# goalheart/ionic-mpnn

Hardware: AMD Instinct MI355X
Metric: molecule-graph pairs/sec (fwd), batch 4096 per MI355X (higher is better)
Workload: dtype f32 (bf16x9 emulation)

## Files before the change

### ionic_mpnn_amd/csrc/encoder_layout.h

```cpp
#pragma once

#include "common.h"

namespace impnn {
namespace enc {

typedef float f32x4 __attribute__((ext_vector_type(4)));
typedef _Float16 half8 __attribute__((ext_vector_type(8)));

constexpr float kSW = 256.0f;
constexpr float kSX = 16.0f;
constexpr float kAcc = kSW * kSX;

constexpr int kD = 32;
constexpr int kKMax = 8;
constexpr int kRCap = 256;
constexpr int kECap = 1024;
constexpr int kHS = 36;
constexpr int kMsgRS = 36;
constexpr int kUpdRS = 68;
constexpr int kThreads = 1024;
constexpr int kWaves = kThreads / 64;
constexpr int kTbCapFloats = 2048;

__host__ __device__ constexpr int img_msg_floats(int K) { return K * kD * kMsgRS; }
__host__ __device__ constexpr int img_upd_floats() { return 3 * kD * kUpdRS; }
__host__ __device__ constexpr int img_vec_floats() { return 5 * kD; }
__host__ __device__ constexpr int img_floats(int K) {
  return img_msg_floats(K) + img_upd_floats() + img_vec_floats();
}
__host__ __device__ constexpr int img16_msg_halfs(int K) { return K * 2 * 2 * 512; }
__host__ __device__ constexpr int img16_upd_halfs() { return 3 * 2 * 2 * 2 * 512; }
__host__ __device__ constexpr int img16_vec_float_off(int K) { return (img16_msg_halfs(K) + img16_upd_halfs()) / 2; }
__host__ __device__ constexpr int feat_of(int q, int j) { return 16 * (j >> 2) + 4 * q + (j & 3); }
constexpr int kPf = 4;
constexpr int kImgSlot = kPf * kThreads * 4;
static_assert(kThreads == 4 * kRCap, "prologue maps 4 threads to a row");
static_assert(img_floats(kKMax) <= kImgSlot, "weight image does not fit its slot");
static_assert(img16_vec_float_off(kKMax) + img_vec_floats() <= kImgSlot, "split weight image does not fit");

constexpr int kRecRowptr = 0;
constexpr int kRecTilemax = 528;
constexpr int kRecMoloff = 544;
constexpr int kRecMolrows = 1072;
constexpr int kRecPoolrow = 1584;
constexpr int kRecRowatom = 2096;
constexpr int kEntMaxAtom = 454;
constexpr int kRecEnt = 3136;
constexpr int kRecBytes = 8192;
static_assert(kRecEnt + 4 * kECap <= kRecBytes && kRecEnt % 16 == 0, "record layout");

constexpr int kTECap = 512;
constexpr int kTECapBig = 640;
__host__ __device__ constexpr int tecap_of(int E) { return E > kTECap ? kTECapBig : kTECap; }
constexpr int kTVbMax = 256;
constexpr int kTHS = 36;
constexpr int kTAS = 32;
constexpr int kTRecRowdeg = 0;
constexpr int kTRecTilemax = 528;
constexpr int kTRecMoloff = 544;
constexpr int kTRecMolrows = 1072;
constexpr int kTRecPoolrow = 1584;
constexpr int kTRecRowatom = 2096;
constexpr int kTRecCounts = 3120;
constexpr int kTRecJdptr = 3136;
constexpr int kTRecNrun = 3664;
constexpr int kTRecGrp = 3712;
constexpr int kTRunTarget = 32;
__host__ __device__ constexpr int tgrp_cap(int Vb, int ecap) { return ecap / 4 + (Vb < kTVbMax ? Vb : kTVbMax); }
__host__ __device__ constexpr int trec_runs_off(int Vb, int ecap) { return kTRecGrp + 16 * tgrp_cap(Vb, ecap); }
__host__ __device__ constexpr int trec_used_bytes(int Vb, int ecap) {
  return (trec_runs_off(Vb, ecap) + 2 * (Vb + 2 + kTRunTarget) + 15) & ~15;
}
constexpr int kTRecBytes = 12288;
constexpr int kTRecPart1 = 8192;
__host__ __device__ constexpr int trec_lds_bytes(int Vb, int ecap) { return trec_used_bytes(Vb, ecap); }
static_assert(kTRecGrp % 16 == 0 && trec_used_bytes(kTVbMax, kTECapBig) <= kTRecBytes, "typed record layout");
__host__ __device__ constexpr int tmsg_floats(int ecap) { return (ecap + 2) * kD; }
__host__ __device__ constexpr int tmsg_off(int s, int u) { return s * kD + ((u ^ ((s >> 1) & 7)) << 2); }
__host__ __device__ constexpr int tmsg_key(int s) { return s * kD + (((s >> 1) & 7) << 2); }
static_assert(tmsg_key(kTECapBig + 1) < 65536, "message keys travel as 16 bits");
constexpr int kTUpdBlocks = 24;
constexpr int kTVecFloatOff = kTUpdBlocks * 256;
constexpr int kTUpdFloats = kTVecFloatOff + 5 * kD;
constexpr int kTUpdSlot = 2 * kThreads * 4;
constexpr int kTUpdLds = 6400;
static_assert(kTUpdFloats <= kTUpdLds && kTUpdLds <= kTUpdSlot, "typed update image");
constexpr int kXUpdHalfs = 3 * 2 * 2 * 3 * 512;
constexpr int kXVecFloatOff = kXUpdHalfs / 2;
constexpr int kXUpdFloats = kXVecFloatOff + 5 * kD;
constexpr int kXUpdSlot = 3 * kThreads * 4;
constexpr int kXUpdLds = 9472;
static_assert(kXUpdFloats <= kXUpdLds && kXUpdLds <= kXUpdSlot, "x3 update image");
constexpr int kTMatFloats = kD * kD;
inline size_t typed_prepared_floats(int S, int Vb, bool x3 = false) {
  const size_t s = S > 0 ? S : 1;
  return s * (x3 ? kXUpdSlot : kTUpdSlot) + s * (size_t)Vb * kTMatFloats + (size_t)Vb * kTMatFloats;
}

constexpr int kShareCap = kECap;
inline int plan_vmin(int n_ions, int B, int vrmax, int nwg) {
  const int64_t span = 2 * (int64_t)n_ions * B * vrmax / (nwg > 0 ? nwg : 1) + vrmax;
  const int64_t v = (span + kShareCap - 2) / (kShareCap - 1);
  return (int)(v < 1 ? 1 : (v > kRCap ? kRCap : v));
}
constexpr int kMaxHops = 128;

constexpr int kPB = 16;

struct Ws {
  size_t img_off, rows_off, vr_off, partial_off, share_off, nsub_off, desc_off, rec_off, total;
  int nwg;
  int max_sub;
  int nblk;
  int rec_bytes;
};

inline size_t align_up(size_t x, size_t a) { return (x + a - 1) / a * a; }

__host__ __device__ constexpr int tvr_of_edges(int edges, int ecap) { return (edges * kRCap + ecap - 1) / ecap; }

inline int vr_max_of(int N, int E, bool typed = false) {
  int v = typed ? (E > 4 * kTECapBig ? kRCap + 1 : tvr_of_edges(E, tecap_of(E))) : (E + 3) / 4;
  int m = N > v ? N : v;
  m = m < 1 ? 1 : m;
  return typed && m > kRCap ? kRCap : m;
}

struct PlanHeader {
  int32_t magic, kind, n_ions, B, N, E, nwg, max_sub;
  int32_t overflow;
};
constexpr int32_t kPlanMagic = 0x696d706e;
constexpr int32_t kPlanBadBit = 1 << 30;

inline Ws ws_layout(int n_ions, int B, int N, int E, int S, int Vb, int nwg, bool typed, bool x3 = false) {
  Ws w{};
  const int vrmax = vr_max_of(N, E, typed);
  w.rec_bytes = typed ? kTRecBytes : kRecBytes;
  const int win = kRCap - vrmax + 1;
  w.nwg = nwg;
  w.nblk = (B + kPB - 1) / kPB;
  const int64_t share_rows = (2 * (int64_t)n_ions * B * vrmax) / nwg + vrmax;
  const int64_t by_win = win >= 1 ? share_rows / win + 2 : (int64_t)1 << 40;
  const int64_t by_pairs = 2 * share_rows / (kRCap + 1) + 2;
  w.max_sub = (int)(by_win < by_pairs ? by_win : by_pairs);
  size_t off = 256;
  w.img_off = off;
  off = align_up(off + (typed ? (size_t)n_ions * typed_prepared_floats(S, Vb, x3)
                              : (size_t)n_ions * (S > 0 ? S : 1) * kImgSlot) * sizeof(float), 256);
  w.rows_off = off;
  off = align_up(off + (size_t)n_ions * B * sizeof(int32_t), 256);
  w.vr_off = off;
  off = align_up(off + (size_t)n_ions * B * sizeof(int32_t), 256);
  w.partial_off = off;
  off = align_up(off + (size_t)n_ions * w.nblk * sizeof(int32_t), 256);
  w.share_off = off;
  off = align_up(off + (size_t)nwg * 4 * sizeof(int32_t), 256);
  w.nsub_off = off;
  off = align_up(off + (size_t)nwg * sizeof(int32_t), 256);
  w.desc_off = off;
  off = align_up(off + (size_t)nwg * w.max_sub * 4 * sizeof(int32_t), 256);
  w.rec_off = off;
  off = align_up(off + (size_t)nwg * w.max_sub * w.rec_bytes, 256);
  w.total = off;
  return w;
}

struct PlanParams {
  const int32_t* atom_ids[2];
  const int32_t* bond_ids[2];
  const int32_t* conn[2];
  int32_t* rows;
  int32_t* vr;
  int32_t* partial;
  int32_t* nsub;
  int32_t* desc;
  unsigned char* rec;
  int n_ions, B, N, E, Va, Vb, nwg, max_sub, nblk;
  int grid_sub;
  int typed;
  int ecap;
  int vmin;
  PlanHeader* header;
  unsigned long long* stamps;
};

struct ImageParams {
  const float* weights;
  float* img;
  int K, mode;
  int64_t step_floats;
};

struct EncParams {
  const int32_t* atom_ids[2];
  float* pooled[2];
  const float* atom_table;
  const float* bond_table;
  const float* img[2];
  const int32_t* nsub;
  const int32_t* desc;
  const unsigned char* rec;
  const PlanHeader* header;
  int n_ions, B, N, K, S, Va, Vb, max_sub;
  int atab_lds;
  float ln_eps;
  unsigned long long* stamps;
};

struct TImageParams {
  const float* weights;
  const float* bond_table;
  float* prepared;
  int K, S, Vb, x3;
  int64_t step_floats;
};

struct TEncParams {
  float* pooled[2];
  const float* atom_table;
  const float* upd[2];
  const float* tmat[2];
  const int32_t* nsub;
  const int32_t* desc;
// ... 36 lines not shown
```

### ionic_mpnn_amd/csrc/encoder_plan.hip

```cpp
#include "encoder_layout.h"

namespace impnn {
namespace enc {

namespace {

__global__ __launch_bounds__(64 * kPB) void plan_stats_kernel(PlanParams p) {
  __shared__ int vsum[kPB], vbad[kPB];
  __builtin_amdgcn_s_setprio(3);
  const int lane = threadIdx.x & 63, wv = threadIdx.x >> 6;
  const int g = blockIdx.x / p.nblk, blk = blockIdx.x - g * p.nblk;
  const int b = blk * kPB + wv;
  const bool have = b < p.B;
  const int64_t item = (int64_t)g * p.B + (have ? b : 0);
  int my_vr = 0, my_bad = 0;
  if (have) {
  const int32_t* ids = p.atom_ids[g] + (int64_t)b * p.N;
  const int32_t* cn = p.conn[g] + (int64_t)b * p.E * 2;
  const int32_t* bd = p.bond_ids[g] + (int64_t)b * p.E;
  int rmax = 0, cnt = 0;
  const int id_first = lane < p.N ? ids[lane] : 0;
  int emax = 0;
  for (int e0 = 0; e0 < p.E; e0 += 256) {
    int2 st[4];
// ... 728 lines not shown
    const int slot = tid + k * kRCap;
    sid[k] = slot < n_ids ? ids_c[slot] : 0;
  }
  for (int m = tid; m <= M; m += kRCap) {
    const int off = T.shst[mb_local + m] - base;
    moloff[m] = off;
    r_moloff[m] = (uint16_t)off;
    if (m < M) {
      const int rr = rows_g[m0 + m];
      molrows[m] = rr;
      r_molrows[m] = (uint16_t)rr;
    }
  }
  cnt[tid] = 0;
  dbins[tid] = 0;
  dcur[tid] = 0;
  thist[tid] = 0;
  tcur[tid] = 0;
  idl[tid] = -1;
  if (tid == 0) misc[1] = 0;
  {
    const uint4 ones = make_uint4(~0u, ~0u, ~0u, ~0u);
    reinterpret_cast<uint4*>(tick)[2 * tid] = ones;
    reinterpret_cast<uint4*>(tick)[2 * tid + 1] = ones;
  }
  lds_barrier();
  CSTAMP(2);

  auto put_id = [&](int slot, int id) {
    const int m = fast_div(slot, N, rN), n = slot - m * N;
    if (slot < n_ids && n < molrows[m]) idl[moloff[m] + n] = id;
  };
  {
    const int dq = fast_div(kRCap, N, rN), dr = kRCap - dq * N;
    int cm = fast_div(tid, N, rN), cn = tid - cm * N;
    int mr[kIC], mo[kIC], nn[kIC];
#pragma unroll
    for (int k = 0; k < kIC; ++k) {
      const int mm = tid + k * kRCap < n_ids ? cm : 0;
      mr[k] = tid + k * kRCap < n_ids ? molrows[mm] : 0;
      mo[k] = moloff[mm];
      nn[k] = cn;
      cn += dr; cm += dq;
      if (cn >= N) { cn -= N; ++cm; }
    }
#pragma unroll
    for (int k = 0; k < kIC; ++k)
      if (nn[k] < mr[k]) idl[mo[k] + nn[k]] = sid[k];
  }
  for (int slot = tid + kIC * kRCap; slot < n_ids; slot += kRCap) put_id(slot, ids_c[slot]);
  {
    unsigned okm = 0u;
#pragma unroll
    for (int k = 0; k < kSC; ++k) okm |= edge_valid(sst[k].x, sst[k].y, sbid[k], N, p.Vb) ? 1u << k : 0u;
    const int mine = __builtin_popcount(okm);
    const int incl = wave_incl_scan(mine);
    int pos = 0;
    if (lane == 63) pos = atomicAdd(&misc[1], incl);
    pos = __builtin_amdgcn_readlane(pos, 63) + incl - mine;
    const int dq = fast_div(kRCap, E, rE), dr = kRCap - dq * E;
    int cm = fast_div(tid, E, rE), ce = tid - cm * E;
#pragma unroll
    for (int k0 = 0; k0 < kSC; k0 += 3) {
      int row[3], srw[3], tk[3], es[3];
#pragma unroll
      for (int k = 0; k < 3; ++k) {
        const bool ok = (okm >> (k0 + k)) & 1u;
        const int m = cm;
        es[k] = ce;
        ce += dr; cm += dq;
        if (ce >= E) { ce -= E; ++cm; }
        const int mo = moloff[m < M ? m : 0];
        row[k] = mo + (ok ? sst[k0 + k].y : 0);
        srw[k] = mo + (ok ? sst[k0 + k].x : 0);
      }
#pragma unroll
      for (int k = 0; k < 3; ++k) {
        const bool ok = (okm >> (k0 + k)) & 1u;
        tk[k] = atomicAdd(&cnt[ok ? row[k] : kRCap + lane], 1);
        atomicAdd(&thist[ok ? sbid[k0 + k] : kTVbMax + lane], 1);
      }
#pragma unroll
      for (int k = 0; k < 3; ++k) {
        const bool ok = (okm >> (k0 + k)) & 1u;
        if (ok && tk[k] < kTick) tick[row[k] * kTick + tk[k]] = (uint16_t)es[k];
        if (ok) {
          if (pos < kTECapBig)
            elist[pos] = make_uint2((uint32_t)row[k] | ((uint32_t)srw[k] << 8) | ((uint32_t)sbid[k0 + k] << 16), (uint32_t)es[k]);
          ++pos;
        }
      }
    }
  }
  for (int s0 = kSC * kRCap; s0 < n_slots; s0 += kRCap) {
    const int slot = s0 + tid;
    int2 st = make_int2(0, 0);
    int bid = -1;
    if (slot < n_slots) {
      st = *reinterpret_cast<const int2*>(conn_c + 2 * (int64_t)slot);
      bid = bond_c[slot];
    }
    const bool ok = edge_valid(st.x, st.y, bid, N, p.Vb);
    const int m = fast_div(slot, E, rE), e = slot - m * E;
    const int mo = moloff[m < M ? m : 0];
    const int row = mo + (ok ? st.y : 0);
    int tk = kTick;
    if (ok) {
      tk = atomicAdd(&cnt[row], 1);
      atomicAdd(&thist[bid], 1);
    }
    const unsigned long long okb = __ballot(ok);
    int pos0 = 0;
    if (okb != 0ull) {
      if (lane == (int)__builtin_ctzll(okb)) pos0 = atomicAdd(&misc[1], (int)__builtin_popcountll(okb));
      pos0 = __builtin_amdgcn_readlane(pos0, (int)__builtin_ctzll(okb));
    }
    if (tk < kTick) tick[row * kTick + tk] = (uint16_t)e;
    const int pos = pos0 + (int)__builtin_popcountll(okb & ((1ull << lane) - 1));
    if (ok && pos < kTECapBig)
      elist[pos] = make_uint2((uint32_t)row | ((uint32_t)(mo + st.x) << 8) | ((uint32_t)bid << 16), (uint32_t)e);
  }
  lds_barrier();
  CSTAMP(3);

  const int my_deg = cnt[tid];
  const int dcl = my_deg > 255 ? 255 : my_deg;
  if (tid < R) {
    if (my_deg > 255) p.header->overflow = 1;
    atomicAdd(&dbins[255 - dcl], 1);
  }
  lds_barrier();
  CSTAMP(4);

  if (wave == 0) {
    const int4 h = reinterpret_cast<const int4*>(dbins)[lane];
    const int s4 = h.x + h.y + h.z + h.w;
    const int ex = wave_incl_scan(s4) - s4;
    reinterpret_cast<int4*>(dstart)[lane] = make_int4(ex, ex + h.x, ex + h.x + h.y, ex + h.x + h.y + h.z);
    __builtin_amdgcn_s_waitcnt(0xc07f);
    const int4 s = reinterpret_cast<const int4*>(dstart)[63 - lane];
    const int t4 = s.x + s.y + s.z + s.w;
    const int incl = wave_incl_scan(t4);
    const int jx = incl - t4;
    reinterpret_cast<int4*>(jdp)[lane] = make_int4(jx, jx + s.w, jx + s.w + s.z, jx + s.w + s.z + s.y);
    if (lane == 63) { jdp[kRCap] = incl; jdp[kRCap + 1] = incl; }
  } else if (wave == 1) {
    const int4 n = reinterpret_cast<const int4*>(thist)[lane];
    const int4 ng = make_int4((n.x + 3) >> 2, (n.y + 3) >> 2, (n.z + 3) >> 2, (n.w + 3) >> 2);
    const int s4 = ng.x + ng.y + ng.z + ng.w;
    const int incl = wave_incl_scan(s4);
    const int ex = incl - s4;
    reinterpret_cast<int4*>(tgb)[lane] = make_int4(ex, ex + ng.x, ex + ng.x + ng.y, ex + ng.x + ng.y + ng.z);
    const int ngrp_all = __builtin_amdgcn_readlane(incl, 63);
    int gmax = (ngrp_all + kTRunTarget - 1) / kTRunTarget;
    gmax = gmax < 2 ? 2 : gmax;
    const float rgm = 1.0f / (float)gmax;
    const int4 nr = make_int4(fast_div(ng.x + gmax - 1, gmax, rgm), fast_div(ng.y + gmax - 1, gmax, rgm),
                              fast_div(ng.z + gmax - 1, gmax, rgm), fast_div(ng.w + gmax - 1, gmax, rgm));
    const int r4 = nr.x + nr.y + nr.z + nr.w;
    const int rincl = wave_incl_scan(r4);
    int ri = rincl - r4;
    uint16_t* runs = reinterpret_cast<uint16_t*>(rec + trec_runs_off(p.Vb, p.ecap));
    for (int i = 0; i < nr.x; ++i) runs[ri++] = (uint16_t)(ex + i * gmax);
    for (int i = 0; i < nr.y; ++i) runs[ri++] = (uint16_t)(ex + ng.x + i * gmax);
    for (int i = 0; i < nr.z; ++i) runs[ri++] = (uint16_t)(ex + ng.x + ng.y + i * gmax);
    for (int i = 0; i < nr.w; ++i) runs[ri++] = (uint16_t)(ex + ng.x + ng.y + ng.z + i * gmax);
    if (lane == 63) {
      runs[rincl] = (uint16_t)incl;
      *reinterpret_cast<uint16_t*>(rec + kTRecNrun) = (uint16_t)rincl;
      misc[0] = incl;
    }
  }
  lds_barrier();
  CSTAMP(5);

  int pos = tid;
  if (tid < R) pos = dstart[255 - dcl] + atomicAdd(&dcur[255 - dcl], 1);
  place[tid] = pos;
  {
    const int my_id = idl[tid];
    r_rowatom[pos] = my_id;
    r_poolrow[tid] = (uint16_t)(pos | (my_id > 0 ? 0x8000 : 0));
    r_rowdeg[pos] = (uint16_t)my_deg;
    if ((pos & 15) == 0) r_tilemax[pos >> 4] = (unsigned char)dcl;
    r_jd[tid] = (uint16_t)jdp[tid];
    if (tid < 2) r_jd[kRCap + tid] = (uint16_t)jdp[kRCap];
    if (pos == 0) {
      r_cw[0] = (uint16_t)misc[0];
      r_cw[1] = (uint16_t)jdp[kRCap];
      r_cw[2] = (uint16_t)dcl;
    }
  }
  {
    const int n_t = thist[tid];
    const int ng = (n_t + 3) >> 2, gb = tgb[tid];
    const uint32_t dump = (uint32_t)tmsg_key(p.ecap) * 0x10001u;
    for (int jg = 0; jg < ng; ++jg) {
      const int c = n_t - 4 * jg;
      grp[gb + jg] = make_uint4((uint32_t)tid | ((uint32_t)(c < 4 ? c : 4) << 8) | ((uint32_t)(ng - jg) << 24), 0u, dump, dump);
    }
  }
  lds_barrier();
  CSTAMP(6);

  {
    auto below = [](uint4 a, uint32_t ue) {
      return (int)(((a.x & 0xffffu) < ue) + ((a.x >> 16) < ue) + ((a.y & 0xffffu) < ue) + ((a.y >> 16) < ue) +
                   ((a.z & 0xffffu) < ue) + ((a.z >> 16) < ue) + ((a.w & 0xffffu) < ue) + ((a.w >> 16) < ue));
    };
    const int nval = misc[1] < kTECapBig ? misc[1] : kTECapBig;
    for (int i0 = 0; i0 < nval; i0 += 2 * kRCap) {
      bool ok[2];
      uint2 en[2];
      int row[2], srow[2], deg[2], ix[2], gb[2], rank[2];
      uint4 ta[2], tb[2];
#pragma unroll
      for (int k = 0; k < 2; ++k) {
        const int i = i0 + k * kRCap + tid;
        ok[k] = i < nval;
        en[k] = elist[ok[k] ? i : 0];
      }
#pragma unroll
      for (int k = 0; k < 2; ++k) {
        const int rt = (int)(en[k].x & 0xffu), bid = (int)(en[k].x >> 16);
        deg[k] = cnt[rt];
        ta[k] = reinterpret_cast<const uint4*>(tick)[2 * rt];
        tb[k] = reinterpret_cast<const uint4*>(tick)[2 * rt + 1];
        row[k] = place[rt];
        srow[k] = place[(en[k].x >> 8) & 0xffu];
        gb[k] = tgb[bid];
        ix[k] = atomicAdd(&tcur[ok[k] ? bid : kTVbMax + lane], 1);
      }
#pragma unroll
      for (int k = 0; k < 2; ++k) {
        rank[k] = below(ta[k], en[k].y) + below(tb[k], en[k].y);
        if (deg[k] > kTick) {
          const int rt = (int)(en[k].x & 0xffu);
          int lo = 0, hi = M - 1;
          while (lo < hi) {
            const int mid = (lo + hi + 1) >> 1;
            if (moloff[mid] <= rt) lo = mid; else hi = mid - 1;
          }
          const int t = rt - moloff[lo];
          const int32_t* cm = conn_c + 2 * (int64_t)lo * E;
          const int32_t* bm = bond_c + (int64_t)lo * E;
          rank[k] = 0;
          for (int e2 = 0; e2 < (int)en[k].y; ++e2) {
            const int2 s2 = *reinterpret_cast<const int2*>(cm + 2 * e2);
            rank[k] += (s2.y == t && edge_valid(s2.x, s2.y, bm[e2], N, p.Vb)) ? 1 : 0;
          }
        }
        rank[k] = jdp[rank[k] < 256 ? rank[k] : 255];
      }
#pragma unroll
      for (int k = 0; k < 2; ++k) {
        if (ok[k]) {
          unsigned char* ge = reinterpret_cast<unsigned char*>(&grp[gb[k] + (ix[k] >> 2)]);
          ge[4 + (ix[k] & 3)] = (unsigned char)srow[k];
          reinterpret_cast<uint16_t*>(ge + 8)[ix[k] & 3] = (uint16_t)tmsg_key(rank[k] + row[k]);
        }
      }
    }
  }
  lds_barrier();
  CSTAMP(9);

  {
    const int ngrp = misc[0];
    uint4* r_grp = reinterpret_cast<uint4*>(rec + kTRecGrp);
    for (int i = tid; i < ngrp; i += kRCap) r_grp[i] = grp[i];
  }
  CSTAMP(15);
  lds_barrier();
  }
}
#undef CSTAMP

}

int launch_weight_image(const ImageParams& ip, int S, hipStream_t s) {
  if (S <= 0) return IMPNN_OK;
  weight_image_kernel<<<dim3(16, S), 256, 0, s>>>(ip);
  return check_launch("weight_image");
}

int launch_typed_image(const TImageParams& ip, hipStream_t s) {
  const int S = ip.S > 0 ? ip.S : 1;
  float* canon = ip.prepared + (size_t)S * (ip.x3 ? kXUpdSlot : kTUpdSlot) + (size_t)S * ip.Vb * kTMatFloats;
  for (int st = 0; st < ip.S; ++st) {
    if (int rc = launch_bond_type_matrices(ip.bond_table, ip.weights + (int64_t)st * ip.step_floats, canon, ip.Vb, ip.K,
                                           kD, s))
      return rc;
    typed_image_kernel<<<(ip.Vb * kTMatFloats + kTUpdSlot + 255) / 256 < 256 ? (ip.Vb * kTMatFloats + kTUpdSlot + 255) / 256 : 256,
                         256, 0, s>>>(ip, st);
    if (int rc = check_launch("typed_image")) return rc;
  }
  return IMPNN_OK;
}

int launch_plan(const PlanParams& pp, hipStream_t s) {
  plan_stats_kernel<<<pp.n_ions * pp.nblk, 64 * kPB, 0, s>>>(pp);
  if (int rc = check_launch("plan_stats")) return rc;
  if ((int64_t)2 * pp.n_ions * pp.B / pp.nwg + 64 > kShareCap)
    return fail(IMPNN_E_UNSUPPORTED, "encoder plan: batch of %d molecules per ion is too large", pp.B);
  if (pp.max_sub > kMaxHops)
    return fail(IMPNN_E_UNSUPPORTED, "encoder plan: %d chunk slots per workgroup", pp.max_sub);
  if (pp.typed)
    plan_chunks_typed_kernel<<<pp.nwg * pp.grid_sub, kRCap, sizeof(uint4) * tgrp_cap(pp.Vb, pp.ecap), s>>>(pp);
  else
    plan_chunks_kernel<<<pp.nwg * pp.grid_sub, kRCap, 0, s>>>(pp);
  return check_launch("plan_chunks");
}

}
}
```

### ionic_mpnn_amd/csrc/encoder_typed.hip

```cpp
#include "encoder_device.h"
#include "encoder_layout.h"

namespace impnn {
namespace enc {

namespace {

constexpr int kOffUpd = 0;
constexpr int off_h(bool x3) { return kOffUpd + (x3 ? kXUpdLds : kTUpdLds); }
constexpr int kTHSBig3 = 32;
constexpr int off_msg(bool x3, int hs = kTHS) { return off_h(x3) + kRCap * hs; }
constexpr int off_rec(bool x3, int ecap, int hs = kTHS) { return off_msg(x3, hs) + tmsg_floats(ecap); }
constexpr size_t lds_fixed_bytes(bool x3, int Vb, int ecap, int hs = kTHS) {
  return sizeof(float) * (size_t)off_rec(x3, ecap, hs) + trec_lds_bytes(Vb, ecap);
}
static_assert(lds_fixed_bytes(true, kTVbMax, kTECap) <= 160 * 1024 && lds_fixed_bytes(false, kTVbMax, kTECapBig) <= 160 * 1024 &&
                  lds_fixed_bytes(true, kTVbMax, kTECapBig, kTHSBig3) <= 160 * 1024,
              "LDS budget");

typedef __bf16 bf16x8 __attribute__((ext_vector_type(8)));
struct B3 {
  bf16x8 p0, p1, p2;
};
__device__ __forceinline__ void split_pair(float x, float y, unsigned& w0, unsigned& w1, unsigned& w2) {
  const unsigned xb = __builtin_bit_cast(unsigned, x), yb = __builtin_bit_cast(unsigned, y);
  const float x1 = x - __builtin_bit_cast(float, xb & 0xffff0000u), y1 = y - __builtin_bit_cast(float, yb & 0xffff0000u);
  const unsigned x1b = __builtin_bit_cast(unsigned, x1), y1b = __builtin_bit_cast(unsigned, y1);
  const float x2 = x1 - __builtin_bit_cast(float, x1b & 0xffff0000u), y2 = y1 - __builtin_bit_cast(float, y1b & 0xffff0000u);
  w0 = __builtin_amdgcn_perm(yb, xb, 0x07060302u);
  w1 = __builtin_amdgcn_perm(y1b, x1b, 0x07060302u);
  w2 = __builtin_amdgcn_perm(__builtin_bit_cast(unsigned, y2), __builtin_bit_cast(unsigned, x2), 0x07060302u);
}
__device__ __forceinline__ B3 split8x3(f32x4 a, f32x4 b) {
  union {
    bf16x8 v;
    unsigned u[4];
  } q0, q1, q2;
  split_pair(a[0], a[1], q0.u[0], q1.u[0], q2.u[0]);
  split_pair(a[2], a[3], q0.u[1], q1.u[1], q2.u[1]);
  split_pair(b[0], b[1], q0.u[2], q1.u[2], q2.u[2]);
  split_pair(b[2], b[3], q0.u[3], q1.u[3], q2.u[3]);
  B3 r;
  r.p0 = q0.v;
  r.p1 = q1.v;
  r.p2 = q2.v;
  return r;
}
__device__ __forceinline__ f32x4 mfmab(bf16x8 a, bf16x8 b, f32x4 c) {
  return __builtin_amdgcn_mfma_f32_16x16x32_bf16(a, b, c, 0, 0, 0);
}
__device__ __forceinline__ void mma9x2(f32x4& c0, f32x4& c1, const __bf16* blk0, const __bf16* blk1, int lane, const B3& b) {
  const bf16x8 a00 = *reinterpret_cast<const bf16x8*>(blk0 + lane * 8);
  const bf16x8 a01 = *reinterpret_cast<const bf16x8*>(blk0 + 512 + lane * 8);
  const bf16x8 a02 = *reinterpret_cast<const bf16x8*>(blk0 + 1024 + lane * 8);
  const bf16x8 a10 = *reinterpret_cast<const bf16x8*>(blk1 + lane * 8);
  const bf16x8 a11 = *reinterpret_cast<const bf16x8*>(blk1 + 512 + lane * 8);
  const bf16x8 a12 = *reinterpret_cast<const bf16x8*>(blk1 + 1024 + lane * 8);
  c0 = mfmab(a02, b.p2, c0);  c1 = mfmab(a12, b.p2, c1);
  c0 = mfmab(a01, b.p2, c0);  c1 = mfmab(a11, b.p2, c1);
  c0 = mfmab(a02, b.p1, c0);  c1 = mfmab(a12, b.p1, c1);
  c0 = mfmab(a00, b.p2, c0);  c1 = mfmab(a10, b.p2, c1);
  c0 = mfmab(a02, b.p0, c0);  c1 = mfmab(a12, b.p0, c1);
  c0 = mfmab(a01, b.p1, c0);  c1 = mfmab(a11, b.p1, c1);
  c0 = mfmab(a00, b.p1, c0);  c1 = mfmab(a10, b.p1, c1);
  c0 = mfmab(a01, b.p0, c0);  c1 = mfmab(a11, b.p0, c1);
  c0 = mfmab(a00, b.p0, c0);  c1 = mfmab(a10, b.p0, c1);
}

template <int ABID>
__device__ __forceinline__ f32x4 mfma1(float a, float b, f32x4 c) {
  return __builtin_amdgcn_mfma_f32_4x4x1f32(a, b, c, 3, ABID, 0);
}

typedef float f32x2v __attribute__((ext_vector_type(2)));
struct Grp {
  uint4 ge;
  f32x2v aq;
};
struct Run {
  f32x4 bq[4];
  Grp first;
};

#ifndef IMPNN_T_PF
#define IMPNN_T_PF 0
#endif
#ifndef IMPNN_T_EARLY
#define IMPNN_T_EARLY 0
#endif
constexpr int kPfWhere = IMPNN_T_PF, kRunsEarly = IMPNN_T_EARLY;

template <bool STAMPS, bool X3, int HS = kTHS>
__global__ __launch_bounds__(kThreads, kThreads / 256) void encoder_typed_kernel(TEncParams p) {
  extern __shared__ __align__(16) float smem[];
  constexpr int kUpdLds = X3 ? kXUpdLds : kTUpdLds, kUpdSlot = X3 ? kXUpdSlot : kTUpdSlot;
  constexpr int kNPf = X3 ? 3 : 2;
  float* const wupd = smem + kOffUpd;
  float* const wvec = wupd + (X3 ? kXVecFloatOff : kTVecFloatOff);
  float* const hbuf = smem + off_h(X3);
  float* const msg = smem + off_msg(X3, HS);
  const int zero_slot = p.ecap + 1;
  unsigned char* const recl = reinterpret_cast<unsigned char*>(smem + off_rec(X3, p.ecap, HS));
  const int rec_lds = p.rec_lds;
  float* const atab = reinterpret_cast<float*>(recl + rec_lds);
  const uint16_t* const r_rowdeg = reinterpret_cast<const uint16_t*>(recl + kTRecRowdeg);
  const unsigned char* const r_tilemax = recl + kTRecTilemax;
  const uint16_t* const r_moloff = reinterpret_cast<const uint16_t*>(recl + kTRecMoloff);
  const uint16_t* const r_molrows = reinterpret_cast<const uint16_t*>(recl + kTRecMolrows);
  const uint16_t* const r_poolrow = reinterpret_cast<const uint16_t*>(recl + kTRecPoolrow);
  const int32_t* const r_rowatom = reinterpret_cast<const int32_t*>(recl + kTRecRowatom);
  const uint16_t* const r_jdptr = reinterpret_cast<const uint16_t*>(recl + kTRecJdptr);
  const uint16_t* const r_runs = reinterpret_cast<const uint16_t*>(recl + trec_runs_off(p.Vb, p.ecap));
  int* const run_ctr = reinterpret_cast<int*>(recl + kTRecCounts + 8);
  const uint4* const r_grp = reinterpret_cast<const uint4*>(recl + kTRecGrp);

  const int tid = threadIdx.x, lane = tid & 63;
  const int wave = __builtin_amdgcn_readfirstlane(tid >> 6);
  const int a = lane & 15, q = lane >> 4;
  unsigned long long* stamp = STAMPS && p.stamps ? p.stamps + (size_t)blockIdx.x * 32 : nullptr;
  if (stamp && tid == 0) stamp[0] = __builtin_amdgcn_s_memtime();

  {
    const PlanHeader hd = *p.header;
    if (hd.magic != kPlanMagic || hd.kind != 1 || hd.nwg != (int)gridDim.x || hd.max_sub != p.max_sub ||
        hd.B != p.B || hd.n_ions != p.n_ions || hd.overflow != 0) {
      const float nan = __builtin_nanf("");
      for (int g = 0; g < p.n_ions; ++g)
        for (int64_t t = (int64_t)blockIdx.x * kThreads + tid; t < (int64_t)p.B * kD; t += (int64_t)gridDim.x * kThreads)
          p.pooled[g][t] = nan;
      return;
    }
  }
  const int c_begin = blockIdx.x * p.max_sub;
  const int c_end = c_begin + __builtin_amdgcn_readfirstlane(p.nsub[blockIdx.x]);
  if (c_begin >= c_end) return;

  if (p.atab_lds)
    for (int t = tid; t < (p.Va + 1) * (kTAS / 4); t += kThreads)
      st4(atab + 4 * t, t < p.Va * (kD / 4) ? ld4(p.atom_table + 4 * t) : f32x4{0.f, 0.f, 0.f, 0.f});
  if (tid < kD) msg[zero_slot * kD + tid] = 0.f;
  unsigned long long t_pro = 0, t_steps = 0, t_pool = 0, t_mark = 0, t_msg = 0;
  if (stamp && tid == 0) t_mark = __builtin_amdgcn_s_memtime();

  auto pool = [&](int M, int m0, int g) {
    float* out_g = p.pooled[g];
    for (int t0 = 0; t0 < M * 64; t0 += kThreads) {
      const int t = t0 + tid;
      const int part = t & 7, f4 = (t >> 3) & 7, m = t >> 6;
      f32x4 acc = {0.f, 0.f, 0.f, 0.f};
      if (m < M) {
        const int nr = r_molrows[m], mo = r_moloff[m];
        for (int n = part; n < nr; n += 8) {
          const int pr = r_poolrow[mo + n];
          if (pr & 0x8000) acc += ld4(hbuf + (pr & 0xff) * HS + 4 * f4);
        }
      }
#pragma unroll
      for (int i = 0; i < 4; ++i) {
        float v = acc[i];
        v += __builtin_bit_cast(float, __builtin_amdgcn_update_dpp(0, __builtin_bit_cast(int, v), 0xb1, 0xf, 0xf, true));
        v += __builtin_bit_cast(float, __builtin_amdgcn_update_dpp(0, __builtin_bit_cast(int, v), 0x4e, 0xf, 0xf, true));
        v += __builtin_bit_cast(float, __builtin_amdgcn_update_dpp(0, __builtin_bit_cast(int, v), 0x141, 0xf, 0xf, true));
        acc[i] = v;
      }
      if (m < M && part == 0) st4(out_g + (int64_t)(m0 + m) * kD + 4 * f4, acc);
    }
  };
  auto fill_h0 = [&]() {
    const int row = tid >> 2, sub = tid & 3;
    const int id = r_rowatom[row];
    f32x4 v0 = {0.f, 0.f, 0.f, 0.f}, v1 = v0;
    if ((unsigned)id < (unsigned)p.Va) {
      if (p.atab_lds) {
        v0 = ld4(atab + id * kTAS + 8 * sub);
        v1 = ld4(atab + id * kTAS + 8 * sub + 4);
      } else {
        v0 = ld4(p.atom_table + (int64_t)id * kD + 8 * sub);
        v1 = ld4(p.atom_table + (int64_t)id * kD + 8 * sub + 4);
      }
    }
    st4(hbuf + row * HS + 8 * sub, v0);
    st4(hbuf + row * HS + 8 * sub + 4, v1);
  };

  if (p.S == 0) {
    for (int c = c_begin; c < c_end; ++c) {
      const unsigned char* rc = p.rec + (size_t)c * kTRecBytes;
      if (8 * tid < rec_lds) reinterpret_cast<uint2*>(recl)[tid] = reinterpret_cast<const uint2*>(rc)[tid];
      const int4 dsc = reinterpret_cast<const int4*>(p.desc)[c];
      lds_barrier();
      fill_h0();
      lds_barrier();
      pool(__builtin_amdgcn_readfirstlane(dsc.y), __builtin_amdgcn_readfirstlane(dsc.x),
           __builtin_amdgcn_readfirstlane(dsc.w) >> 16);
      lds_barrier();
    }
    return;
  }

  const bool rec_big = rec_lds > kTRecPart1;
  const unsigned char* rec_c = p.rec + (size_t)c_begin * kTRecBytes;
  uint2 rec_n8 = reinterpret_cast<const uint2*>(rec_c)[tid];
  uint32_t rec_n4 = rec_big ? reinterpret_cast<const uint32_t*>(rec_c + kTRecPart1)[tid] : 0u;
  int4 dsc_next = reinterpret_cast<const int4*>(p.desc)[c_begin];

  const uint32_t* const grp_x = reinterpret_cast<const uint32_t*>(r_grp);
  const int kh = lane >> 5, f = lane & 31;
  const int boff = kh * 512 + f * 4;
  const int ysh = 8 * (lane & 3), zsh = 16 * kh;
  const int acol = 16 * kh + 2 * ((lane >> 2) & 7);

  for (int c = c_begin; c < c_end; ++c) {
    const int4 dsc = dsc_next;
    const int m0 = __builtin_amdgcn_readfirstlane(dsc.x), M = __builtin_amdgcn_readfirstlane(dsc.y);
    const int rg = __builtin_amdgcn_readfirstlane(dsc.w);
    const int R = rg & 0xffff, g = rg >> 16;
    const int ntiles = (R + 15) >> 4;
    const float* upd_g = p.upd[g];
    const float* tmat_g = p.tmat[g];
    if (8 * tid < rec_lds) reinterpret_cast<uint2*>(recl)[tid] = rec_n8;
    if (rec_big && kTRecPart1 + 4 * tid < rec_lds) reinterpret_cast<uint32_t*>(recl + kTRecPart1)[tid] = rec_n4;
    {
      const int cn = (c + 1) < c_end ? (c + 1) : c;
      const unsigned char* rn = p.rec + (size_t)cn * kTRecBytes;
      rec_n8 = reinterpret_cast<const uint2*>(rn)[tid];
      if (rec_big) rec_n4 = reinterpret_cast<const uint32_t*>(rn + kTRecPart1)[tid];
      dsc_next = reinterpret_cast<const int4*>(p.desc)[cn];
    }
    lds_barrier();
    fill_h0();
    if (tid == 0) *run_ctr = 2 * kWaves;
    lds_barrier();
    if (stamp && tid == 0) {
      const unsigned long long t = __builtin_amdgcn_s_memtime();
      t_pro += t - t_mark;
      t_mark = t;
    }
    const int nrun = __builtin_amdgcn_readfirstlane(*reinterpret_cast<const uint16_t*>(recl + kTRecNrun));

    Run P, Q;
    int gP = 0, nP = 0, gQ = 0, nQ = 0;
    bool haveP = false, haveQ = false;
    const bool sP = wave < nrun, sQ = wave + kWaves < nrun;
    const int sgP = __builtin_amdgcn_readfirstlane(r_runs[sP ? wave : 0]);
    const int snP = __builtin_amdgcn_readfirstlane(r_runs[(sP ? wave : 0) + 1]) - sgP;
    const int sgQ = __builtin_amdgcn_readfirstlane(r_runs[sQ ? wave + kWaves : 0]);
    const int snQ = __builtin_amdgcn_readfirstlane(r_runs[(sQ ? wave + kWaves : 0) + 1]) - sgQ;
    const int soP = sP ? (__builtin_amdgcn_readfirstlane(grp_x[4 * sgP]) & 0xff) * kTMatFloats : 0;
    const int soQ = sQ ? (__builtin_amdgcn_readfirstlane(grp_x[4 * sgQ]) & 0xff) * kTMatFloats : 0;
    const int lboffP = sP ? boff : 0, lboffQ = sQ ? boff : 0;
    f32x4 pf[kNPf];
    auto fetch_pf = [&](int s_) {
#pragma unroll
      for (int i = 0; i < kNPf; ++i) pf[i] = ld4(upd_g + (int64_t)s_ * kUpdSlot + 4 * (tid + i * kThreads));
    };
    auto fetch_P = [&](int s_) {
      const float* tm = tmat_g + (size_t)s_ * p.Vb * kTMatFloats;
#pragma unroll
      for (int i = 0; i < 4; ++i) P.bq[i] = ld4(tm + soP + lboffP + i * 128);
    };
    auto fetch_Q = [&](int s_) {
      const float* tm = tmat_g + (size_t)s_ * p.Vb * kTMatFloats;
#pragma unroll
      for (int i = 0; i < 4; ++i) Q.bq[i] = ld4(tm + soQ + lboffQ + i * 128);
    };
    if (kPfWhere != 0) fetch_pf(0);
    if (kRunsEarly >= 1) fetch_P(0);
    if (kRunsEarly >= 2) fetch_Q(0);
    for (int s = 0; s < p.S; ++s) {
      const float* tm_s = tmat_g + (size_t)s * p.Vb * kTMatFloats;
      __builtin_amdgcn_s_setprio(2);
      {
        const float* const abase = hbuf + acol;
        auto load_group = [&](int e, Grp& G) {
          G.ge = r_grp[e];
          const int src = __builtin_amdgcn_ubfe(G.ge.y, ysh, 8);
          G.aq = *reinterpret_cast<const f32x2v*>(abase + src * HS);
        };
        auto compute = [&](const Grp& G, const f32x4 (&bq)[4]) {
          f32x4 acc0 = {0.f, 0.f, 0.f, 0.f}, acc1 = acc0;
#ifndef IMPNN_DIAG_NO_MSG_MFMA
          acc0 = mfma1<0>(G.aq[0], bq[0][0], acc0);
          acc1 = mfma1<0>(G.aq[1], bq[0][1], acc1);
          acc0 = mfma1<1>(G.aq[0], bq[0][2], acc0);
          acc1 = mfma1<1>(G.aq[1], bq[0][3], acc1);
          acc0 = mfma1<2>(G.aq[0], bq[1][0], acc0);
          acc1 = mfma1<2>(G.aq[1], bq[1][1], acc1);
          acc0 = mfma1<3>(G.aq[0], bq[1][2], acc0);
          acc1 = mfma1<3>(G.aq[1], bq[1][3], acc1);
          acc0 = mfma1<4>(G.aq[0], bq[2][0], acc0);
          acc1 = mfma1<4>(G.aq[1], bq[2][1], acc1);
          acc0 = mfma1<5>(G.aq[0], bq[2][2], acc0);
          acc1 = mfma1<5>(G.aq[1], bq[2][3], acc1);
          acc0 = mfma1<6>(G.aq[0], bq[3][0], acc0);
          acc1 = mfma1<6>(G.aq[1], bq[3][1], acc1);
          acc0 = mfma1<7>(G.aq[0], bq[3][2], acc0);
          acc1 = mfma1<7>(G.aq[1], bq[3][3], acc1);
#else
          acc0[0] = G.aq[0] + bq[0][0] + bq[3][3];
          acc1[1] = G.aq[1] + bq[1][1] + bq[2][2];
#endif
          float x0 = acc0[0] + acc1[0], x1 = acc0[1] + acc1[1], x2 = acc0[2] + acc1[2], x3 = acc0[3] + acc1[3];
          asm volatile("s_nop 1\n\tv_permlane32_swap_b32 %0, %1\n\tv_permlane32_swap_b32 %2, %3"
                       : "+v"(x0), "+v"(x1), "+v"(x2), "+v"(x3));
          msg[__builtin_amdgcn_ubfe(G.ge.z, zsh, 16) ^ f] = x0 + x1;
          msg[__builtin_amdgcn_ubfe(G.ge.w, zsh, 16) ^ f] = x2 + x3;
        };
        auto run_type = [&](int g_, int n_, Run& Rn) {
          const int end = g_ + n_;
          Grp T;
          int e = g_;
          while (true) {
            if (e + 1 < end) load_group(e + 1, T);
            compute(Rn.first, Rn.bq);
            if (++e >= end) break;
            if (e + 1 < end) load_group(e + 1, Rn.first);
            compute(T, Rn.bq);
            if (++e >= end) break;
          }
        };
        auto fetch = [&](bool have, int r, int& g_, int& n_, Run& Rn, const float* tm) {
          const int rc = have ? r : 0;
          g_ = __builtin_amdgcn_readfirstlane(r_runs[rc]);
          n_ = __builtin_amdgcn_readfirstlane(r_runs[rc + 1]) - g_;
          const int type = have ? (__builtin_amdgcn_readfirstlane(grp_x[4 * g_]) & 0xff) : 0;
          const float* bp = tm + (size_t)type * kTMatFloats + (have ? boff : 0);
#pragma unroll
          for (int i = 0; i < 4; ++i) Rn.bq[i] = ld4(bp + i * 128);
        };
        auto next_run = [&]() {
          int r = 0;
          if (lane == 0) r = atomicAdd(run_ctr, 1);
          return __builtin_amdgcn_readfirstlane(r);
        };
        auto take = [&](int r, int& g_, int& n_, Run& Rn) {
          fetch(true, r, g_, n_, Rn, tm_s);
          load_group(g_, Rn.first);
        };
        auto landed = [](f32x4 (&b)[4]) {
          asm volatile("" : "+v"(b[0]), "+v"(b[1]), "+v"(b[2]), "+v"(b[3]) : : "memory");
        };
        if (kPfWhere == 0) fetch_pf(s);
        if (kRunsEarly < 1) fetch_P(s);
        if (kRunsEarly < 2) fetch_Q(s);
        haveP = sP; gP = sgP; nP = snP;
        haveQ = sQ; gQ = sgQ; nQ = snQ;
        if (haveP) load_group(gP, P.first);
        if (haveQ) load_group(gQ, Q.first);
        if (haveP) {
          if (!haveQ) {
            landed(P.bq);
            run_type(gP, nP, P);
          } else {
            while (true) {
              landed(P.bq);
              run_type(gP, nP, P);
              const int rP = next_run();
              if (rP >= nrun) {
                landed(Q.bq);
                run_type(gQ, nQ, Q);
                break;
              }
              take(rP, gP, nP, P);
              landed(Q.bq);
              run_type(gQ, nQ, Q);
              const int rQ = next_run();
              if (rQ >= nrun) {
                landed(P.bq);
                run_type(gP, nP, P);
                break;
              }
              take(rQ, gQ, nQ, Q);
            }
          }
        }
      }
#pragma unroll
      for (int i = 0; i < kNPf; ++i)
        if (4 * (tid + i * kThreads) < kUpdLds) st4(wupd + 4 * (tid + i * kThreads), pf[i]);
      const bool mstamp = stamp && c == c_begin && s == 1;
      if (mstamp && lane == 0) stamp[16 + wave] = __builtin_amdgcn_s_memtime();
      lds_barrier();
      if (tid == 0) *run_ctr = 2 * kWaves;
      if (mstamp && tid == 0) stamp[12] = __builtin_amdgcn_s_memtime();
      if (stamp && tid == 0 && c == c_begin && s == 1) t_msg = __builtin_amdgcn_s_memtime();

      int my_tile = -1;
      {
        const int grp = wave & 3, slot = wave >> 2, q4 = ntiles >> 2, r4 = ntiles & 3;
        const int heavy = (4 - r4) * q4;
        if (grp >= r4) {
          if (slot < q4) my_tile = slot * (4 - r4) + (grp - r4);
        } else if (slot <= q4) {
          my_tile = heavy + slot * r4 + grp;
        }
      }
      const bool has_tile = my_tile >= 0 && my_tile < ntiles;
      if (has_tile) {
        const int tile = my_tile;
        const int row = tile * 16 + a;
        const int deg = r_rowdeg[row];
        const int maxdeg = __builtin_amdgcn_readfirstlane(r_tilemax[tile]);
        f32x4 agg0 = {0.f, 0.f, 0.f, 0.f}, agg1 = agg0;
        for (int d0 = 0; d0 < maxdeg; d0 += 4) {
          const uint2 jd = *reinterpret_cast<const uint2*>(r_jdptr + d0);
          int sl[4];
          sl[0] = d0 + 0 < deg ? (int)(jd.x & 0xffffu) + row : zero_slot;
          sl[1] = d0 + 1 < deg ? (int)(jd.x >> 16) + row : zero_slot;
          sl[2] = d0 + 2 < deg ? (int)(jd.y & 0xffffu) + row : zero_slot;
          sl[3] = d0 + 3 < deg ? (int)(jd.y >> 16) + row : zero_slot;
          f32x4 m0v[4], m1v[4];
#pragma unroll
          for (int j = 0; j < 4; ++j) {
            const int o = tmsg_off(sl[j], q);
            m0v[j] = ld4(msg + o);
            m1v[j] = ld4(msg + (o ^ 16));
          }
#pragma unroll
          for (int j = 0; j < 4; ++j) {
            agg0 += m0v[j];
            agg1 += m1v[j];
          }
        }
        if (mstamp && wave == 1 && lane == 0) stamp[8] = __builtin_amdgcn_s_memtime();
        __builtin_amdgcn_s_setprio(1);
        if (s + 1 < p.S) {
          if (kPfWhere == 1) fetch_pf(s + 1);
          if (kRunsEarly >= 1) fetch_P(s + 1);
          if (kRunsEarly >= 2) fetch_Q(s + 1);
        }
        const f32x4 h0 = ld4(hbuf + row * HS + 4 * q);
        const f32x4 h1 = ld4(hbuf + row * HS + 16 + 4 * q);

        f32x4 z0 = ld4(wvec + 0 * kD + 4 * q), z1 = ld4(wvec + 0 * kD + 16 + 4 * q);
        f32x4 r0 = ld4(wvec + 1 * kD + 4 * q), r1 = ld4(wvec + 1 * kD + 16 + 4 * q);
        f32x4 t0 = ld4(wvec + 2 * kD + 4 * q), t1 = ld4(wvec + 2 * kD + 16 + 4 * q);
        if constexpr (X3) {
          const __bf16* wb = reinterpret_cast<const __bf16*>(wupd);
          const B3 sh = split8x3(h0, h1);
          const B3 sa = split8x3(agg0, agg1);
          mma9x2(z0, z1, wb + ((0 * 2 + 0) * 2 + 0) * 1536, wb + ((0 * 2 + 1) * 2 + 0) * 1536, lane, sh);
          mma9x2(r0, r1, wb + ((1 * 2 + 0) * 2 + 0) * 1536, wb + ((1 * 2 + 1) * 2 + 0) * 1536, lane, sh);
          mma9x2(z0, z1, wb + ((0 * 2 + 0) * 2 + 1) * 1536, wb + ((0 * 2 + 1) * 2 + 1) * 1536, lane, sa);
          mma9x2(r0, r1, wb + ((1 * 2 + 0) * 2 + 1) * 1536, wb + ((1 * 2 + 1) * 2 + 1) * 1536, lane, sa);
          z0 = sigmoid4<false>(z0);
          z1 = sigmoid4<false>(z1);
          const f32x4 rh0 = sigmoid4<false>(r0) * h0;
          const f32x4 rh1 = sigmoid4<false>(r1) * h1;
          const B3 srh = split8x3(rh0, rh1);
          mma9x2(t0, t1, wb + ((2 * 2 + 0) * 2 + 0) * 1536, wb + ((2 * 2 + 1) * 2 + 0) * 1536, lane, srh);
          mma9x2(t0, t1, wb + ((2 * 2 + 0) * 2 + 1) * 1536, wb + ((2 * 2 + 1) * 2 + 1) * 1536, lane, sa);
        } else {
          const float* wl = wupd + 4 * lane;
#pragma unroll
          for (int half = 0; half < 2; ++half) {
#pragma unroll
            for (int u = 0; u < 2; ++u) {
              const int hu = half * 2 + u;
              const f32x4 Az0 = ld4(wl + ((0 * 2 + 0) * 4 + hu) * 256);
              const f32x4 Az1 = ld4(wl + ((0 * 2 + 1) * 4 + hu) * 256);
              const f32x4 Ar0 = ld4(wl + ((1 * 2 + 0) * 4 + hu) * 256);
              const f32x4 Ar1 = ld4(wl + ((1 * 2 + 1) * 4 + hu) * 256);
              const f32x4 Bv = half == 0 ? (u == 0 ? h0 : h1) : (u == 0 ? agg0 : agg1);
#pragma unroll
              for (int r = 0; r < 4; ++r) {
                z0 = mfma4(Az0[r], Bv[r], z0);
                z1 = mfma4(Az1[r], Bv[r], z1);
                r0 = mfma4(Ar0[r], Bv[r], r0);
                r1 = mfma4(Ar1[r], Bv[r], r1);
              }
            }
          }
          z0 = sigmoid4<false>(z0);
          z1 = sigmoid4<false>(z1);
          const f32x4 rh0 = sigmoid4<false>(r0) * h0;
          const f32x4 rh1 = sigmoid4<false>(r1) * h1;
#pragma unroll
          for (int half = 0; half < 2; ++half) {
#pragma unroll
            for (int u = 0; u < 2; ++u) {
              const int hu = half * 2 + u;
              const f32x4 Ah0 = ld4(wl + ((2 * 2 + 0) * 4 + hu) * 256);
              const f32x4 Ah1 = ld4(wl + ((2 * 2 + 1) * 4 + hu) * 256);
              const f32x4 Bv = half == 0 ? (u == 0 ? rh0 : rh1) : (u == 0 ? agg0 : agg1);
#pragma unroll
              for (int r = 0; r < 4; ++r) {
                t0 = mfma4(Ah0[r], Bv[r], t0);
                t1 = mfma4(Ah1[r], Bv[r], t1);
              }
            }
          }
        }
        __builtin_amdgcn_s_setprio(0);
        if (kPfWhere == 2 && s + 1 < p.S) {
          asm volatile("" ::: "memory");
          fetch_pf(s + 1);
        }
        if (mstamp && wave == 1 && lane == 0) stamp[9] = __builtin_amdgcn_s_memtime();
        f32x4 n0 = z0 * (tanh4<false>(t0) - h0) + h0;
        f32x4 n1 = z1 * (tanh4<false>(t1) - h1) + h1;
        const f32x4 s4 = n0 + n1;
        float sum = (s4[0] + s4[1]) + (s4[2] + s4[3]);
        sum += __shfl_xor(sum, 16);
        sum += __shfl_xor(sum, 32);
        const float mean = sum * (1.0f / kD);
        n0 -= mean;
        n1 -= mean;
        const f32x4 q4 = n0 * n0 + n1 * n1;
        float var = (q4[0] + q4[1]) + (q4[2] + q4[3]);
        var += __shfl_xor(var, 16);
        var += __shfl_xor(var, 32);
        const float inv = __builtin_amdgcn_rsqf(var * (1.0f / kD) + p.ln_eps);
        const f32x4 gm0 = ld4(wvec + 3 * kD + 4 * q), gm1 = ld4(wvec + 3 * kD + 16 + 4 * q);
        const f32x4 bt0 = ld4(wvec + 4 * kD + 4 * q), bt1 = ld4(wvec + 4 * kD + 16 + 4 * q);
        const f32x4 o0 = n0 * (gm0 * inv) + (bt0 + h0);
        const f32x4 o1 = n1 * (gm1 * inv) + (bt1 + h1);
        st4(hbuf + row * HS + 4 * q, o0);
        st4(hbuf + row * HS + 16 + 4 * q, o1);
        if (mstamp && wave == 1 && lane == 0) stamp[10] = __builtin_amdgcn_s_memtime();
      }
      if (!has_tile && s + 1 < p.S) {
        if (kPfWhere != 0) fetch_pf(s + 1);
        if (kRunsEarly >= 1) fetch_P(s + 1);
        if (kRunsEarly >= 2) fetch_Q(s + 1);
      }
// ... 113 lines not shown
```

Baseline: 35.44 million.

## Pack run descriptors into 32-bit words and prefetch the next run ticket

Run descriptors change from 16-bit group starts to 32-bit words that pack first group, group count and bond type, with the type field laid out as the matrix byte offset. This removes the dependent LDS read of the group header that the old code needed to find the type, and the second read of the next run start. The dynamic scheduler now pulls the next ticket one run ahead with atomicInc, overlapping the atomic latency with the current run's loads. It uses a zero sentinel word and a larger runs array, and adds asm barriers to keep some address arithmetic in vector registers.

```diff
diff --git a/ionic_mpnn_amd/csrc/encoder_layout.h b/ionic_mpnn_amd/csrc/encoder_layout.h
--- a/ionic_mpnn_amd/csrc/encoder_layout.h
+++ b/ionic_mpnn_amd/csrc/encoder_layout.h
@@ -67,10 +67,25 @@
 constexpr int kTRecNrun = 3664;
 constexpr int kTRecGrp = 3712;
 constexpr int kTRunTarget = 32;
-__host__ __device__ constexpr int tgrp_cap(int Vb, int ecap) { return ecap / 4 + (Vb < kTVbMax ? Vb : kTVbMax); }
+constexpr int kTRunGrpBits = 12, kTRunTypeBits = 8;
+__host__ __device__ constexpr int tgrp_cap(int Vb, int ecap) { return (ecap + 3 * (Vb < kTVbMax ? Vb : kTVbMax)) / 4; }
+__host__ __device__ constexpr int trun_gmax(int groups) {
+  return (groups + kTRunTarget - 1) / kTRunTarget < 2 ? 2 : (groups + kTRunTarget - 1) / kTRunTarget;
+}
+__host__ __device__ constexpr uint32_t trun_word(int first_group, int groups, int type) {
+  return (uint32_t)first_group | ((uint32_t)type << kTRunGrpBits) | ((uint32_t)groups << (kTRunGrpBits + kTRunTypeBits));
+}
+__host__ __device__ constexpr int trun_first(uint32_t w) { return (int)(w & ((1u << kTRunGrpBits) - 1)); }
+__host__ __device__ constexpr int trun_groups(uint32_t w) { return (int)(w >> (kTRunGrpBits + kTRunTypeBits)); }
+__host__ __device__ constexpr uint32_t trun_mat_bytes(uint32_t w) { return w & (((1u << kTRunTypeBits) - 1) << kTRunGrpBits); }
+static_assert(kTECapBig <= 640 && tgrp_cap(kTVbMax, kTECapBig) <= (1 << kTRunGrpBits), "first group of a run: 12 bits");
+static_assert(kTVbMax <= (1 << kTRunTypeBits), "bond type of a run: 8 bits");
+static_assert(trun_gmax(tgrp_cap(kTVbMax, kTECapBig)) < (1 << (32 - kTRunGrpBits - kTRunTypeBits)), "groups of a run: 12 bits");
+static_assert(4 * kD * kD == (1 << kTRunGrpBits), "the type field of a run word is the matrix's byte offset");
+__host__ __device__ constexpr int trun_cap(int Vb) { return (Vb < kTVbMax ? Vb : kTVbMax) + kTRunTarget + 1; }
 __host__ __device__ constexpr int trec_runs_off(int Vb, int ecap) { return kTRecGrp + 16 * tgrp_cap(Vb, ecap); }
 __host__ __device__ constexpr int trec_used_bytes(int Vb, int ecap) {
-  return (trec_runs_off(Vb, ecap) + 2 * (Vb + 2 + kTRunTarget) + 15) & ~15;
+  return (trec_runs_off(Vb, ecap) + 4 * trun_cap(Vb) + 15) & ~15;
 }
 constexpr int kTRecBytes = 12288;
 constexpr int kTRecPart1 = 8192;
diff --git a/ionic_mpnn_amd/csrc/encoder_plan.hip b/ionic_mpnn_amd/csrc/encoder_plan.hip
--- a/ionic_mpnn_amd/csrc/encoder_plan.hip
+++ b/ionic_mpnn_amd/csrc/encoder_plan.hip
@@ -904,21 +904,26 @@
     const int ex = incl - s4;
     reinterpret_cast<int4*>(tgb)[lane] = make_int4(ex, ex + ng.x, ex + ng.x + ng.y, ex + ng.x + ng.y + ng.z);
     const int ngrp_all = __builtin_amdgcn_readlane(incl, 63);
-    int gmax = (ngrp_all + kTRunTarget - 1) / kTRunTarget;
-    gmax = gmax < 2 ? 2 : gmax;
+    const int gmax = trun_gmax(ngrp_all);
     const float rgm = 1.0f / (float)gmax;
     const int4 nr = make_int4(fast_div(ng.x + gmax - 1, gmax, rgm), fast_div(ng.y + gmax - 1, gmax, rgm),
                               fast_div(ng.z + gmax - 1, gmax, rgm), fast_div(ng.w + gmax - 1, gmax, rgm));
     const int r4 = nr.x + nr.y + nr.z + nr.w;
     const int rincl = wave_incl_scan(r4);
     int ri = rincl - r4;
-    uint16_t* runs = reinterpret_cast<uint16_t*>(rec + trec_runs_off(p.Vb, p.ecap));
-    for (int i = 0; i < nr.x; ++i) runs[ri++] = (uint16_t)(ex + i * gmax);
-    for (int i = 0; i < nr.y; ++i) runs[ri++] = (uint16_t)(ex + ng.x + i * gmax);
-    for (int i = 0; i < nr.z; ++i) runs[ri++] = (uint16_t)(ex + ng.x + ng.y + i * gmax);
-    for (int i = 0; i < nr.w; ++i) runs[ri++] = (uint16_t)(ex + ng.x + ng.y + ng.z + i * gmax);
+    uint32_t* runs = reinterpret_cast<uint32_t*>(rec + trec_runs_off(p.Vb, p.ecap));
+    auto cut = [&](int first, int groups, int nruns, int type) {
+      for (int i = 0; i < nruns; ++i) {
+        const int left = groups - i * gmax;
+        runs[ri++] = trun_word(first + i * gmax, left < gmax ? left : gmax, type);
+      }
+    };
+    cut(ex, ng.x, nr.x, 4 * lane);
+    cut(ex + ng.x, ng.y, nr.y, 4 * lane + 1);
+    cut(ex + ng.x + ng.y, ng.z, nr.z, 4 * lane + 2);
+    cut(ex + ng.x + ng.y + ng.z, ng.w, nr.w, 4 * lane + 3);
     if (lane == 63) {
-      runs[rincl] = (uint16_t)incl;
+      runs[rincl] = 0u;
       *reinterpret_cast<uint16_t*>(rec + kTRecNrun) = (uint16_t)rincl;
       misc[0] = incl;
     }
diff --git a/ionic_mpnn_amd/csrc/encoder_typed.hip b/ionic_mpnn_amd/csrc/encoder_typed.hip
--- a/ionic_mpnn_amd/csrc/encoder_typed.hip
+++ b/ionic_mpnn_amd/csrc/encoder_typed.hip
@@ -110,8 +110,8 @@
   const uint16_t* const r_poolrow = reinterpret_cast<const uint16_t*>(recl + kTRecPoolrow);
   const int32_t* const r_rowatom = reinterpret_cast<const int32_t*>(recl + kTRecRowatom);
   const uint16_t* const r_jdptr = reinterpret_cast<const uint16_t*>(recl + kTRecJdptr);
-  const uint16_t* const r_runs = reinterpret_cast<const uint16_t*>(recl + trec_runs_off(p.Vb, p.ecap));
-  int* const run_ctr = reinterpret_cast<int*>(recl + kTRecCounts + 8);
+  const uint32_t* const r_runs = reinterpret_cast<const uint32_t*>(recl + trec_runs_off(p.Vb, p.ecap));
+  unsigned* const run_ctr = reinterpret_cast<unsigned*>(recl + kTRecCounts + 8);
   const uint4* const r_grp = reinterpret_cast<const uint4*>(recl + kTRecGrp);
 
   const int tid = threadIdx.x, lane = tid & 63;
@@ -175,8 +175,10 @@
         v0 = ld4(atab + id * kTAS + 8 * sub);
         v1 = ld4(atab + id * kTAS + 8 * sub + 4);
       } else {
-        v0 = ld4(p.atom_table + (int64_t)id * kD + 8 * sub);
-        v1 = ld4(p.atom_table + (int64_t)id * kD + 8 * sub + 4);
+        int col = 8 * sub;
+        asm volatile("" : "+v"(col));
+        v0 = ld4(p.atom_table + (int64_t)id * kD + col);
+        v1 = ld4(p.atom_table + (int64_t)id * kD + col + 4);
       }
     }
     st4(hbuf + row * HS + 8 * sub, v0);
@@ -204,7 +206,6 @@
   uint32_t rec_n4 = rec_big ? reinterpret_cast<const uint32_t*>(rec_c + kTRecPart1)[tid] : 0u;
   int4 dsc_next = reinterpret_cast<const int4*>(p.desc)[c_begin];
 
-  const uint32_t* const grp_x = reinterpret_cast<const uint32_t*>(r_grp);
   const int kh = lane >> 5, f = lane & 31;
   const int boff = kh * 512 + f * 4;
   const int ysh = 8 * (lane & 3), zsh = 16 * kh;
@@ -242,27 +243,29 @@
     int gP = 0, nP = 0, gQ = 0, nQ = 0;
     bool haveP = false, haveQ = false;
     const bool sP = wave < nrun, sQ = wave + kWaves < nrun;
-    const int sgP = __builtin_amdgcn_readfirstlane(r_runs[sP ? wave : 0]);
-    const int snP = __builtin_amdgcn_readfirstlane(r_runs[(sP ? wave : 0) + 1]) - sgP;
-    const int sgQ = __builtin_amdgcn_readfirstlane(r_runs[sQ ? wave + kWaves : 0]);
-    const int snQ = __builtin_amdgcn_readfirstlane(r_runs[(sQ ? wave + kWaves : 0) + 1]) - sgQ;
-    const int soP = sP ? (__builtin_amdgcn_readfirstlane(grp_x[4 * sgP]) & 0xff) * kTMatFloats : 0;
-    const int soQ = sQ ? (__builtin_amdgcn_readfirstlane(grp_x[4 * sgQ]) & 0xff) * kTMatFloats : 0;
-    const int lboffP = sP ? boff : 0, lboffQ = sQ ? boff : 0;
+    const uint32_t swP = __builtin_amdgcn_readfirstlane(r_runs[sP ? wave : 0]);
+    const uint32_t swQ = __builtin_amdgcn_readfirstlane(r_runs[sQ ? wave + kWaves : 0]);
+    auto static_rows = [&](bool have, uint32_t w, const float* tm) {
+      return tm + (have ? (int)(trun_mat_bytes(w) >> 2) + boff : 0);
+    };
     f32x4 pf[kNPf];
     auto fetch_pf = [&](int s_) {
-#pragma unroll
-      for (int i = 0; i < kNPf; ++i) pf[i] = ld4(upd_g + (int64_t)s_ * kUpdSlot + 4 * (tid + i * kThreads));
+      int t4 = 4 * tid;
+      asm volatile("" : "+v"(t4));
+#pragma unroll
+      for (int i = 0; i < kNPf; ++i) pf[i] = ld4(upd_g + (int64_t)s_ * kUpdSlot + t4 + 4 * i * kThreads);
     };
     auto fetch_P = [&](int s_) {
       const float* tm = tmat_g + (size_t)s_ * p.Vb * kTMatFloats;
-#pragma unroll
-      for (int i = 0; i < 4; ++i) P.bq[i] = ld4(tm + soP + lboffP + i * 128);
+      const float* bp = static_rows(sP, swP, tm);
+#pragma unroll
+      for (int i = 0; i < 4; ++i) P.bq[i] = ld4(bp + i * 128);
     };
     auto fetch_Q = [&](int s_) {
       const float* tm = tmat_g + (size_t)s_ * p.Vb * kTMatFloats;
-#pragma unroll
-      for (int i = 0; i < 4; ++i) Q.bq[i] = ld4(tm + soQ + lboffQ + i * 128);
+      const float* bp = static_rows(sQ, swQ, tm);
+#pragma unroll
+      for (int i = 0; i < 4; ++i) Q.bq[i] = ld4(bp + i * 128);
     };
     if (kPfWhere != 0) fetch_pf(0);
     if (kRunsEarly >= 1) fetch_P(0);
@@ -319,23 +322,27 @@
             if (++e >= end) break;
           }
         };
-        auto fetch = [&](bool have, int r, int& g_, int& n_, Run& Rn, const float* tm) {
-          const int rc = have ? r : 0;
-          g_ = __builtin_amdgcn_readfirstlane(r_runs[rc]);
-          n_ = __builtin_amdgcn_readfirstlane(r_runs[rc + 1]) - g_;
-          const int type = have ? (__builtin_amdgcn_readfirstlane(grp_x[4 * g_]) & 0xff) : 0;
-          const float* bp = tm + (size_t)type * kTMatFloats + (have ? boff : 0);
+        auto ticket = [&]() {
+          unsigned t = 0;
+          if (lane == 0) t = atomicInc(run_ctr, 0xffffffffu);
+          return t;
+        };
+        auto word_of = [&](unsigned t) { return r_runs[t < (unsigned)nrun ? t : (unsigned)nrun]; };
+        auto draw = [&]() { return word_of(ticket()); };
+        auto held = [](uint32_t wv) {
+          asm volatile("" : "+v"(wv));
+          return (uint32_t)__builtin_amdgcn_readfirstlane(wv);
+        };
+        auto take = [&](uint32_t w, int& g_, int& n_, Run& Rn) {
+          unsigned t = ticket();
+          g_ = trun_first(w);
+          n_ = trun_groups(w);
+          const float* bp = reinterpret_cast<const float*>(reinterpret_cast<const char*>(tm_s) + trun_mat_bytes(w)) + boff;
 #pragma unroll
           for (int i = 0; i < 4; ++i) Rn.bq[i] = ld4(bp + i * 128);
-        };
-        auto next_run = [&]() {
-          int r = 0;
-          if (lane == 0) r = atomicAdd(run_ctr, 1);
-          return __builtin_amdgcn_readfirstlane(r);
-        };
-        auto take = [&](int r, int& g_, int& n_, Run& Rn) {
-          fetch(true, r, g_, n_, Rn, tm_s);
           load_group(g_, Rn.first);
+          asm volatile("" : "+v"(t));
+          return word_of(t);
         };
         auto landed = [](f32x4 (&b)[4]) {
           asm volatile("" : "+v"(b[0]), "+v"(b[1]), "+v"(b[2]), "+v"(b[3]) : : "memory");
@@ -343,8 +350,8 @@
         if (kPfWhere == 0) fetch_pf(s);
         if (kRunsEarly < 1) fetch_P(s);
         if (kRunsEarly < 2) fetch_Q(s);
-        haveP = sP; gP = sgP; nP = snP;
-        haveQ = sQ; gQ = sgQ; nQ = snQ;
+        haveP = sP; gP = trun_first(swP); nP = trun_groups(swP);
+        haveQ = sQ; gQ = trun_first(swQ); nQ = trun_groups(swQ);
         if (haveP) load_group(gP, P.first);
         if (haveQ) load_group(gQ, Q.first);
         if (haveP) {
@@ -352,25 +359,24 @@
             landed(P.bq);
             run_type(gP, nP, P);
           } else {
+            uint32_t ahead = draw();
             while (true) {
               landed(P.bq);
               run_type(gP, nP, P);
-              const int rP = next_run();
-              if (rP >= nrun) {
+              if (__builtin_amdgcn_readfirstlane(ahead) == 0u) {
                 landed(Q.bq);
                 run_type(gQ, nQ, Q);
                 break;
               }
-              take(rP, gP, nP, P);
+              ahead = take(held(ahead), gP, nP, P);
               landed(Q.bq);
               run_type(gQ, nQ, Q);
-              const int rQ = next_run();
-              if (rQ >= nrun) {
+              if (__builtin_amdgcn_readfirstlane(ahead) == 0u) {
                 landed(P.bq);
                 run_type(gP, nP, P);
                 break;
               }
-              take(rQ, gQ, nQ, Q);
+              ahead = take(held(ahead), gQ, nQ, Q);
             }
           }
         }
```

Result: no change. 35.56 million (median of 6 runs) (+0.3%).
